# Yasas1994/Jaeger

Measured on AMD Instinct MI355X. Metric: Mbp/s classified (1500bp frags), higher is better.
Workload: dtype f16x3 (split-f16, f32 accumulate)

## Files before the change

include/jaeger_hip.h:

```cpp
#ifndef JAEGER_HIP_H
#define JAEGER_HIP_H

#include <stdint.h>

#ifdef __cplusplus
extern "C" {
#endif

#define JG_ABI_VERSION 1
#define JG_MAX_STAGES 8
#define JG_MAX_BUFS 6
#define JG_MAX_VECS 12

typedef enum {
  JG_OK = 0,
  JG_ERR_INVALID = -1,
  JG_ERR_HIP = -2,
  JG_ERR_UNSUPPORTED = -3,
  JG_ERR_NOMEM = -4,
  JG_ERR_IO = -5
} jg_status;

enum { JG_PTR_HOST = 0, JG_PTR_DEVICE = 1 };

// ... 59 lines not shown
  int32_t padding;
  int32_t mask_mode;
  int32_t in_vec, out_vec;
  int32_t vec_off;
  int32_t arg;
  int64_t w_off;
  int64_t b_off;
  float f0;
  int32_t n_stages;
  jg_stage stages[JG_MAX_STAGES];
} jg_op;

typedef struct jg_engine jg_engine;
typedef struct jg_model jg_model;

int jg_abi_version(void);
int jg_sizeof(int which);
const char *jg_last_error(void);
int jg_engine_create(int device_id, jg_engine **out);
int jg_engine_destroy(jg_engine *e);
int jg_engine_sync(jg_engine *e);
enum { JG_OPT_STREAM_BYTES = 1, JG_OPT_CONV_PC = 2, JG_OPT_TERMINI_EXACT = 3, JG_OPT_DUST_ON_COPY_STREAM = 4,
       JG_OPT_TABLE_NET_LDS = 5, JG_OPT_RESET_PROGRESS = 6, JG_OPT_FUSE_RESBLOCK = 7, JG_OPT_TERMINI_REPORT_MIN = 8,
       JG_OPT_STREAM_PRIORITY = 9 };
int jg_engine_set_option(jg_engine *e, int key, int64_t value);
enum { JG_STAT_STREAM_GROUPS = 1, JG_STAT_STREAM_BYTES = 2, JG_STAT_PEAK_DEVICE_BASES = 3, JG_STAT_DUST_MASKED = 4,
       JG_STAT_WINDOWS_DONE = 5 };
int64_t jg_engine_get_stat(const jg_engine *e, int key);
int jg_engine_set_dust(jg_engine *e, const int64_t *rec_off, int64_t n_records, int32_t window, int32_t threshold);

int jg_model_create(jg_engine *e, const jg_op *ops, int n_ops, const float *weights,
                    int64_t n_weights, int32_t vocab, jg_model **out);
int jg_model_destroy(jg_model *m);
int jg_model_set_precision(jg_model *m, int mode);
int jg_model_get_precision(const jg_model *m);
enum { JG_MSTAT_CONVS = 0, JG_MSTAT_CONVS_F16X3 = 1, JG_MSTAT_LAYOUT_CONVERSIONS = 2, JG_MSTAT_SMALL_FUSED = 3,
       JG_MSTAT_TAP_VARIANT = 4 };
int64_t jg_model_get_stat(const jg_model *m, int key);
enum { JG_TAP_F16S = 1, JG_TAP_PHASE_SPLIT = 2, JG_TAP_WINDOW_PACKED = 4, JG_TAP_TABLE_LOOKUP = 8, JG_TAP_NARROW = 16,
       JG_TAP_EXACT_F32 = 32, JG_TAP_FUSED_RESBLOCK = 64 };
int jg_model_tap_shape(const jg_model *m, int op, int32_t l, int64_t shape[4]);
int jg_model_set_tap(jg_model *m, int op, void *host_dst, int64_t dst_bytes);
int jg_model_describe(const jg_model *m, char *buf, int64_t cap);

enum { JG_ENC_PRECASED = 1, JG_ENC_CASE_SENSITIVE = 2, JG_ENC_NUCLEOTIDE = 4, JG_ENC_DICODON = 8 };
int jg_encode(jg_engine *e, const uint8_t *bases, int64_t n_bases, int bases_loc,
              const int64_t *win_start, const int32_t *win_len, int win_loc, int64_t n_win,
              int32_t fsize, const uint8_t *lut65, int32_t soft_mask, int32_t l_pad,
              uint8_t *ids, int32_t *counts, int out_loc, void *stream);

int jg_forward(jg_model *m, const uint8_t *ids, int ids_loc, int64_t n_win, int32_t l,
               float *prediction, float *reliability, float *embedding, float *nmd,
               int out_loc, int32_t chunk, void *stream);

int jg_predict_windows(jg_model *m, const uint8_t *bases, int64_t n_bases, int bases_loc,
                       const int64_t *win_start, const int32_t *win_len, int win_loc,
                       int64_t n_win, int32_t fsize, const uint8_t *lut65, int32_t soft_mask,
                       int32_t l_pad, float *prediction, float *reliability, float *embedding,
                       float *nmd, int32_t *counts, int out_loc, int32_t chunk, void *stream);

// ... 64 lines not shown
```

jaeger_amd/_lib.py:

```python

from __future__ import annotations

import ctypes as C
import os
from pathlib import Path

JG_MAX_STAGES = 8
JG_MAX_BUFS = 6
JG_MAX_VECS = 12
JG_PTR_HOST, JG_PTR_DEVICE = 0, 1
JG_BUF_NONE, JG_BUF_IDS = -1, -2
JG_OK, JG_ERR_INVALID, JG_ERR_HIP, JG_ERR_UNSUPPORTED, JG_ERR_NOMEM, JG_ERR_IO = 0, -1, -2, -3, -4, -5
JG_OPT_STREAM_BYTES = 1
JG_OPT_CONV_PC = 2
JG_OPT_TERMINI_EXACT = 3
JG_OPT_TERMINI_REPORT_MIN = 8
JG_OPT_DUST_ON_COPY_STREAM = 4
JG_OPT_TABLE_NET_LDS = 5
JG_OPT_RESET_PROGRESS = 6
JG_OPT_FUSE_RESBLOCK = 7
JG_OPT_STREAM_PRIORITY = 9
JG_COL_STRING, JG_COL_INT, JG_COL_FLOAT, JG_COL_BOOL, JG_COL_SPANS = 0, 1, 2, 3, 4
JG_STAT_STREAM_GROUPS, JG_STAT_STREAM_BYTES, JG_STAT_PEAK_DEVICE_BASES, JG_STAT_DUST_MASKED, JG_STAT_WINDOWS_DONE = 1, 2, 3, 4, 5
JG_MSTAT_CONVS, JG_MSTAT_CONVS_F16X3, JG_MSTAT_LAYOUT_CONVERSIONS, JG_MSTAT_SMALL_FUSED = 0, 1, 2, 3
JG_MSTAT_TAP_VARIANT = 4
JG_PROF_MFMA_F16X3, JG_PROF_MFMA_F32, JG_PROF_TABLE, JG_PROF_FUSED_SMALL, JG_PROF_FRAMEATTN, JG_PROF_FRAMEATTN_CVT = range(6)
TAP_F16S, TAP_PHASE_SPLIT, TAP_WINDOW_PACKED, TAP_TABLE_LOOKUP, TAP_NARROW, TAP_EXACT_F32, TAP_FUSED_RESBLOCK = 1, 2, 4, 8, 16, 32, 64

OP_CONV, OP_MASK, OP_POOL, OP_DENSE, OP_ELTWISE, OP_NMD_FINAL, OP_OODSIG, OP_MAXPOOL1D, OP_FRAMESUM, OP_STRANDS, OP_EMBED, OP_VECMAX, OP_FRAMEATTN = range(1, 14)
ST_NONE, ST_BIAS, ST_BN, ST_DYT, ST_ADD, ST_ACT, ST_NMD, ST_MASKMUL, ST_LN = range(9)
ACT_NONE, ACT_GELU_TANH, ACT_GELU_ERF, ACT_RELU, ACT_TANH, ACT_SIGMOID = range(6)
MASK_ANY, MASK_MAJORITY, MASK_STRICT = range(3)
PAD_VALID, PAD_SAME = 0, 1
POOL_MAX, POOL_AVG, POOL_MAX_NOMASK = 0, 1, 2
MERGE_AVERAGE, MERGE_SUM, MERGE_MAX, MERGE_CONCAT = 0, 1, 2, 3
JG_ENC_PRECASED, JG_ENC_CASE_SENSITIVE, JG_ENC_NUCLEOTIDE, JG_ENC_DICODON = 1, 2, 4, 8
VEC_EMBEDDING, VEC_NMD, VEC_PREDICTION, VEC_RELIABILITY, VEC_SCRATCH0 = 0, 1, 2, 3, 4


class JgStage(C.Structure):
    _fields_ = [("kind", C.c_int32), ("arg", C.c_int32),
                ("p0", C.c_int64), ("p1", C.c_int64), ("p2", C.c_int64), ("p3", C.c_int64),
                ("f0", C.c_float), ("pad_", C.c_int32)]


class JgOp(C.Structure):
    _fields_ = [("kind", C.c_int32), ("in_buf", C.c_int32), ("out_buf", C.c_int32),
                ("in_mask", C.c_int32), ("out_mask", C.c_int32),
# ... 117 lines not shown
```

jaeger_amd/csrc/jg_api.hip:

```cpp
#include <stdarg.h>
#include <stdio.h>
#include <string.h>

#include <algorithm>
#include <string>
#include <thread>

#include "jg_common.h"
#include "jg_small.h"
#include "jg_resblock64.h"
#include "jg_vecmax.h"
#include "jg_frameattn.h"

static thread_local char g_err[1024] = "";

void jg_set_error(const char *fmt, ...) {
  va_list ap;
  va_start(ap, fmt);
  vsnprintf(g_err, sizeof(g_err), fmt, ap);
  va_end(ap);
}

extern "C" const char *jg_last_error(void) { return g_err; }
extern "C" int jg_abi_version(void) { return JG_ABI_VERSION; }
// ... 66 lines not shown
#ifndef JG_EXPERIMENT
      JG_REQUIRE(value == 0, JG_ERR_UNSUPPORTED, "jg_engine_set_option: JG_OPT_CONV_PC = %lld needs the experiment build (make -C jaeger_amd/csrc "
                 "exp; JAEGER_HIP_LIB=jaeger_amd/libjaeger_hip_exp.so): the producer / consumer kernels are not in the shipped library",
                 (long long)value);
#endif
      e->conv_pc = (int)value;
      return JG_OK;
    case JG_OPT_TERMINI_EXACT:
      e->termini_exact = value != 0;
      return JG_OK;
    case JG_OPT_TERMINI_REPORT_MIN:
      JG_REQUIRE(value == 0 || (value >= 2 && value <= 15), JG_ERR_INVALID,
                 "jg_engine_set_option: JG_OPT_TERMINI_REPORT_MIN = %lld (0, or 2 .. 15 columns)", (long long)value);
      e->termini_report_min = (int)value;
      return JG_OK;
    case JG_OPT_DUST_ON_COPY_STREAM:
      e->dust_on_copy = value != 0;
      return JG_OK;
    case JG_OPT_TABLE_NET_LDS:
      e->tab_lds_only = value != 0;
      return JG_OK;
    case JG_OPT_FUSE_RESBLOCK:
      e->fuse_resblock = value != 0;
      return JG_OK;
    case JG_OPT_RESET_PROGRESS:
      e->windows_done.store(0, std::memory_order_release);
      return JG_OK;
    case JG_OPT_STREAM_PRIORITY: {
      JG_REQUIRE(value == 0 || value == 1, JG_ERR_INVALID, "jg_engine_set_option: JG_OPT_STREAM_PRIORITY takes 0 or 1, got %lld",
                 (long long)value);
      JG_HIP(hipSetDevice(e->dev));
      JG_HIP(hipStreamSynchronize(e->stream));
      int least = 0, greatest = 0;
      JG_HIP(hipDeviceGetStreamPriorityRange(&least, &greatest));
      hipStream_t fresh = nullptr;
      JG_HIP(hipStreamCreateWithPriority(&fresh, hipStreamNonBlocking, value ? greatest : least));
      (void)hipStreamDestroy(e->stream);
      e->stream = fresh;
      return JG_OK;
    }
    default:
      jg_set_error("jg_engine_set_option: unknown key %d", key);
      return JG_ERR_INVALID;
  }
}

// ... 1337 lines not shown
    out += line;
  }
  const size_t n = std::min(out.size(), (size_t)cap - 1);
  memcpy(buf, out.data(), n);
  buf[n] = 0;
  return JG_OK;
}

extern "C" int64_t jg_model_get_stat(const jg_model *m, int key) {
  if (m == nullptr) return -1;
  int64_t n_conv = 0, n_f16 = 0, n_cvt = 0;
  for (size_t i = 0; i < m->ops.size(); ++i) {
    n_cvt += m->hprep[i].n_cvt;
    if (m->ops[i].kind != JG_OP_CONV) continue;
    ++n_conv;
    n_f16 += (m->f16_eligible && m->hprep[i].f16_ok) ? 1 : 0;
  }
  switch (key) {
    case JG_MSTAT_CONVS: return n_conv;
    case JG_MSTAT_CONVS_F16X3: return n_f16;
    case JG_MSTAT_LAYOUT_CONVERSIONS: return m->f16_eligible ? n_cvt : 0;
    case JG_MSTAT_SMALL_FUSED: return m->small != nullptr ? 1 : 0;
    case JG_MSTAT_TAP_VARIANT: return m->tap_variant;
    default: return -1;
  }
}

extern "C" int jg_model_destroy(jg_model *m);
extern "C" int jg_model_create(jg_engine *e, const jg_op *ops, int n_ops, const float *weights,
                               int64_t n_weights, int32_t vocab, jg_model **out) {
  JG_REQUIRE(e != nullptr && ops != nullptr && n_ops > 0 && weights != nullptr && n_weights > 0 &&
                 out != nullptr,
             JG_ERR_INVALID, "jg_model_create: bad arguments");
  JG_HIP(hipSetDevice(e->dev));
  jg_model *m = new jg_model();
  m->e = e;
  m->ops.assign(ops, ops + n_ops);
  m->n_w = n_weights;
  m->vocab = vocab;
  int rc = validate_program(m);
  if (rc != JG_OK) { delete m; return rc; }
  if (m->ops[0].kind == JG_OP_EMBED && m->vocab > 256) m->id_bytes = 2;
  if (m->ops.back().kind == JG_OP_STRANDS) {
    m->strands = m->ops.back().k;
    m->id_frames = 1;
    m->merge_kind = m->ops.back().arg;
// ... 493 lines not shown
              a.wh = hp.d_wh_ps[in.L & 1];
              a.tap_lo = 1; a.tap_hi = 3;
              a.pad_left = 1 + a.tap_lo * a.dil;
            } else {
              a.tap_lo = a.tap_hi = 2;
              a.pad_left = 0 + a.tap_lo * a.dil;
            }
          }
          a.psplit = hp.ps_store ? 1 : 0;
          a.L_res = eff_stride == 2 ? 2 * lo - 1 : lo;
          a.tiles_m = (a.L_res + jg_conv_f16_tile_m() - 1) / jg_conv_f16_tile_m();
          const int strips = hp.cw == 128 ? 2 : 4;
          int strips_per_win = in.frames * a.tiles_m * strips;
          {
            static const bool no_flat = jg_exp_env("JG_NO_FLAT") != nullptr;
            const int halo = (a.k - 1) * a.dil;
            const int gap = std::max(a.pad_left, halo - a.pad_left);
            const int fp = lo + gap;
            const bool strip_rows = hp.nmd_slot >= 0 || hp.nmd_slot2 >= 0 || hp.pool_op >= 0;
            const int wp_unit = strip_rows ? 128 : 32;
            const int wp = (in.frames * fp + wp_unit - 1) / wp_unit * wp_unit;
            const int64_t flat_tiles = ((int64_t)nw * wp + 255) / 256;
            const int64_t row_tiles = (int64_t)a.rows * a.tiles_m;
            if (!no_flat && a.k == 5 && op.in_buf != JG_BUF_IDS && hp.d_lut == nullptr && eff_stride == 1 && eff_lin == lo &&
                ((op.cout == 128 && !hp.as_k5 && hp.ps_read == 0 && !hp.ps_store) ? jg_conv_f16_has_flat_pattern(hp.ep) : jg_conv_f16_has_narrow_pattern(hp.ep)) &&
                (int64_t)nw * wp < (1 << 24) && flat_tiles * 100 <= row_tiles * 95) {
              a.flat = 1;
              a.flat_p = fp;
              a.flat_wp = wp;
              a.flat_frames = in.frames;
              a.flat_tiles = (int)flat_tiles;
              a.flat_inv_p = 1.0f / (float)fp;
              a.flat_inv_wp = 1.0f / (float)wp;
              strips_per_win = wp / (256 / strips);
              m->tap_flat = 1;
            }
          }
          if (hp.nmd_slot >= 0) m->part_rows[hp.nmd_slot] = strips_per_win;
          if (hp.nmd_slot2 >= 0) m->part_rows[hp.nmd_slot2] = strips_per_win;
          if (hp.pool_op >= 0) m->pool_rows = strips_per_win;
          a.out_f16s = hp.out_f16s ? 1 : 0;
          a.act_kind = hp.act_kind;
          a.n_hst = hp.n_hst;
          a.ep = hp.ep;
          a.alpha1 = hp.alpha1; a.alpha2 = hp.alpha2;
          a.dytmask1 = hp.dytmask1; a.dytmask2 = hp.dytmask2;
          a.n_epi_rows = hp.n_epi_rows;
          a.epi = hp.d_epi;
          for (int q = 0; q < hp.n_hst; ++q) a.hst[q] = hp.hst[q];
          if (hp.add_slot >= 0) a.addh = reinterpret_cast<const uint4 *>(m->act[hp.add_slot]);
          if (hp.nmd_slot >= 0) a.nmd_out = m->nmd_part[hp.nmd_slot];
          if (hp.nmd_slot2 >= 0) a.nmd_out2 = m->nmd_part[hp.nmd_slot2];
          a.ep_rt = hp.ep_rt;
          if (hp.pool_op >= 0) {
            const int64_t need = (int64_t)a.rows * a.tiles_m * strips * op.cout;
            if (need > m->pool_part_cap) {
              JG_HIP(hipStreamSynchronize(s));
              if (m->pool_part) (void)hipFree(m->pool_part);
// ... 258 lines not shown
      return rc;
    if (m->precision != 1) break;
    int flag = 0;
    JG_HIP(hipMemcpyAsync(&flag, m->d_overflow, sizeof(int), hipMemcpyDeviceToHost, s));
    JG_HIP(hipStreamSynchronize(s));
    if (flag == 0) break;
    JG_HIP(hipMemsetAsync(m->d_overflow, 0, sizeof(int), s));
    m->precision = 0;
    m->f16_reason = "an activation left the f16 range at run time";
  }
  return JG_OK;
}

extern "C" int jg_forward(jg_model *m, const uint8_t *ids, int ids_loc, int64_t n_win, int32_t l,
                          float *prediction, float *reliability, float *embedding, float *nmd,
                          int out_loc, int32_t chunk, void *stream) {
  JG_REQUIRE(m != nullptr && ids != nullptr && n_win >= 0 && l > 0, JG_ERR_INVALID,
             "jg_forward: bad arguments");
  if (n_win == 0) return JG_OK;
  jg_engine *e = m->e;
  JG_HIP(hipSetDevice(e->dev));
  hipStream_t s = pick_stream(e, stream);
  m->tap_variant = 0;
  const uint8_t *d_ids = ids;
  if (ids_loc == JG_PTR_HOST) {
    const int64_t bytes = n_win * m->strands * m->id_frames * (int64_t)l * m->id_bytes;
    int rc = grow(&m->d_ids, &m->d_ids_cap, bytes);
    if (rc != JG_OK) return rc;
    JG_HIP(hipMemcpyAsync(m->d_ids, ids, (size_t)bytes, hipMemcpyHostToDevice, s));
    d_ids = m->d_ids;
  }
  int rc = forward_device_ids(m, d_ids, n_win, l, prediction, reliability, embedding, nmd, out_loc,
                              chunk, s);
  if (rc != JG_OK) return rc;
  if (out_loc == JG_PTR_HOST || ids_loc == JG_PTR_HOST) JG_HIP(hipStreamSynchronize(s));
  return JG_OK;
}

static int frame_len(int nt) {
  if (nt < 3) return 0;
  const int off = (nt % 3 == 0) ? -2 : ((nt % 3 == 1) ? -1 : 0);
  const int usable = nt - 5 + off;
  return usable > 0 ? (usable + 2) / 3 : 0;
}

static int encode_common(jg_engine *e, jg_model *scratch_owner, const uint8_t *bases, int64_t n_bases,
// ... 428 lines not shown
```

jaeger_amd/csrc/jg_common.h:

```cpp
#pragma once
#include <hip/hip_runtime.h>
#include <stdint.h>
#include <atomic>
#include <string>
#include <vector>

#include "jaeger_hip.h"

void jg_set_error(const char *fmt, ...);

#include <stdlib.h>
static inline const char *jg_exp_env(const char *name) {
#ifdef JG_EXPERIMENT
  return getenv(name);
#else
  (void)name;
  return nullptr;
#endif
}

#define JG_HIP(call)                                                                 \
  do {                                                                               \
    hipError_t err_ = (call);                                                        \
    if (err_ != hipSuccess) {                                                        \
// ... 128 lines not shown
struct ProfEvent {
  hipEvent_t a, b;
  double flops;
  int cls = 0;
};

struct jg_engine {
  int dev = 0;
  hipStream_t stream = nullptr;
  hipEvent_t t0 = nullptr, t1 = nullptr;
  bool profile = false;
  std::vector<ProfEvent> pending;
  std::vector<hipEvent_t> pool;
  double conv_ms = 0.0, conv_flops = 0.0;
  int64_t conv_launches = 0;
  double cls_ms[JG_PROF_CLASSES] = {}, cls_flops[JG_PROF_CLASSES] = {};
  int64_t cls_launches[JG_PROF_CLASSES] = {};
  int n_cu = 256;
  int dust_on_copy = 1;
  int termini_exact = 0;
  int termini_report_min = 0;
  int tab_lds_only = 0;
  int fuse_resblock = 1;
  int conv_pc = 0;
  int64_t stream_bytes = (int64_t)32 << 20;
  hipStream_t copy_stream = nullptr;
  void *pin[2] = {nullptr, nullptr};
  void *dbase[2] = {nullptr, nullptr};
  int64_t pin_cap = 0, dbase_cap = 0;
  hipEvent_t h2d_done[2] = {nullptr, nullptr};
  hipEvent_t enc_done[2] = {nullptr, nullptr};
  hipEvent_t grp_done[2] = {nullptr, nullptr};
  void *pin_io[2] = {nullptr, nullptr};
  int64_t pin_io_cap = 0;
  std::atomic<int64_t> windows_done{0};
  int64_t streamed_groups = 0, streamed_bytes = 0, peak_dev_bases = 0;
  int64_t *d_rec_off = nullptr;
  int64_t rec_cap = 0, n_rec = 0, rec_end = 0;
  int dust_window = 0, dust_threshold = 0;
  unsigned long long *d_dust_cnt = nullptr;
};

struct ConvHPrep {
  uint4 *d_wh = nullptr;
  int n_half = 1;
  int cw = 128;
// ... 69 lines not shown
  uint8_t *d_lut = nullptr;
  float *pool_part = nullptr;
  int64_t pool_part_cap = 0;
  std::vector<int> pool_fused_by;
  int strands = 1;
  int id_frames = 6;
  int id_bytes = 1;
  int merge_kind = 0;
  float *merged[JG_MAX_VECS] = {};
  int64_t merged_cap[JG_MAX_VECS] = {};
  float *tab_table = nullptr;
  float *tab_bias = nullptr;
  int tab_conv = -1, tab_pool = -1;
  uint16_t *tab_wfrag = nullptr;
  float *tab_bias512 = nullptr;
  int tab_act = 0, tab_cq = 0, tab_vocab = 0, tab_zero = 0;
  int part_rows[JG_MAX_BUFS] = {};
  int pool_rows = 0;
  int tap_op = -1;
  void *tap_dst = nullptr;
  int64_t tap_bytes = 0;
  int64_t tap_row0 = 0;
  int64_t tap_variant = 0;
  int tap_flat = 0;
  float *tap_buf = nullptr;
  int64_t tap_cap = 0;
};

int jg_usable_cores();

int jg_launch_conv(jg_engine *e, const ConvArgs &a, hipStream_t s);
int jg_launch_embed(const uint16_t *ids, int64_t n_pos, const float *table, int vocab, int c, float *out, uint8_t *mask,
                    hipStream_t s);
int jg_launch_mask(const uint8_t *in, int rows, int L_in, int L_out, int k, int stride, int dil,
                   int pad_left, int mode, uint8_t *out, hipStream_t s);
int jg_launch_pool(const float *x, const uint8_t *mask, int n_win, int positions, int c, int kind,
                   float *out, int out_ld, hipStream_t s);
int jg_launch_dense(const float *in, int in_ld, const float *w, const float *b, int n_win, int cin,
                    int cout, int act, float *out, int out_ld, hipStream_t s);
int jg_launch_nmd_final(const float *part, int parts_per_win, const uint8_t *mask, int positions,
                        const float *moving_mean, float eps, int n_win, int c, float *out,
                        int out_ld, int out_off, hipStream_t s);
int jg_launch_eltwise(const EltArgs &a, hipStream_t s);
int jg_launch_layernorm(const EltArgs &a, int rows, int L, int tiles_m, hipStream_t s);
int jg_launch_encode(const uint8_t *bases, const int64_t *win_start, const int32_t *win_len,
                     int64_t n_win, int fsize, const uint8_t *lut, int flags, int l_pad,
// ... 47 lines not shown
```

jaeger_amd/csrc/jg_conv_dev.h:

```cpp
#pragma once
#include "jg_common.h"

typedef float f32x16 __attribute__((ext_vector_type(16)));
typedef _Float16 half8 __attribute__((ext_vector_type(8)));
typedef _Float16 half4 __attribute__((ext_vector_type(4)));

namespace {

constexpr int HM = 256;
constexpr int HN = 128;
constexpr int HT = 256;
constexpr int NT = 1;
constexpr int A_ITERS = 5;
constexpr int W_ITERS = 2;
constexpr int W_ITEMS = 2 * 2 * HN;
constexpr int LUT_RS = 68;

__device__ __forceinline__ float fast_gelu(float v) {
  const float t = v * (-2.3022082f - 0.10294324f * v * v);
  return v * __builtin_amdgcn_rcpf(1.0f + __builtin_amdgcn_exp2f(t));
}
typedef float f32x2 __attribute__((ext_vector_type(2)));
__device__ __forceinline__ f32x2 fast_gelu2(f32x2 v) {
  const f32x2 c2 = {0.10294324f, 0.10294324f}, c1 = {-2.3022082f, -2.3022082f}, one = {1.0f, 1.0f};
// ... 57 lines not shown
template <int N>
__device__ __forceinline__ void wait_vm() {
  asm volatile("s_waitcnt vmcnt(%0)" ::"n"(N) : "memory");
}

template <int H>
__device__ __forceinline__ float mix_sum(unsigned hi2, unsigned lo2) {
  float r;
  if constexpr (H == 0) asm("v_fma_mix_f32 %0, %1, 1.0, %2 op_sel:[0,0,0] op_sel_hi:[1,0,1]" : "=v"(r) : "v"(hi2), "v"(lo2));
  else asm("v_fma_mix_f32 %0, %1, 1.0, %2 op_sel:[1,0,1] op_sel_hi:[1,0,1]" : "=v"(r) : "v"(hi2), "v"(lo2));
  return r;
}
template <int H>
__device__ __forceinline__ float mix_rem(float v, unsigned hi2) {
  float r;
  if constexpr (H == 0) asm("v_fma_mix_f32 %0, %1, -1.0, %2 op_sel:[0,0,0] op_sel_hi:[1,0,0]" : "=v"(r) : "v"(hi2), "v"(v));
  else asm("v_fma_mix_f32 %0, %1, -1.0, %2 op_sel:[1,0,0] op_sel_hi:[1,0,0]" : "=v"(r) : "v"(hi2), "v"(v));
  return r;
}

struct Tile {
  int rowblk, m0, valid;
  int T;
};

__device__ __forceinline__ void udivmod24(int v, int d, float inv, int &q, int &r) {
  q = (int)((float)v * inv);
  r = v - q * d;
  if (r < 0) { --q; r += d; }
  else if (r >= d) { ++q; r -= d; }
}

}
```

jaeger_amd/csrc/jg_conv_f16_impl.h:

```cpp
#include <stdio.h>
#include <stdlib.h>
#include <type_traits>

#include "jg_common.h"

#include "jg_conv_dev.h"

namespace {


#ifdef JG_STAMP
static __device__ unsigned long long jg_stamp_acc[8];
#define JG_ST_DECL unsigned long long st_[8] = {0, 0, 0, 0, 0, 0, 0, 0}; unsigned long long st_t = __builtin_amdgcn_s_memtime(); const unsigned long long st_t0 = st_t
#define JG_ST(idx) do { const unsigned long long n_ = __builtin_amdgcn_s_memtime(); st_[idx] += n_ - st_t; st_t = n_; } while (0)
#define JG_ST_END do { st_[5] = __builtin_amdgcn_s_memtime() - st_t0; if (lane == 0) { for (int q_ = 0; q_ < 8; ++q_) atomicAdd(&jg_stamp_acc[q_], st_[q_]); } } while (0)
#else
#define JG_ST_DECL
#define JG_ST(idx)
#define JG_ST_END
#endif

#ifndef JG_PRIO
#define JG_PRIO 1
#endif
// ... 27 lines not shown
  const int wm = LUT ? (wid & 1) : (NARROW ? wid : (wid >> 1));
  const int wn = LUT ? ((GEN && a.lut_one_half) ? 0 : (int)(blockIdx.x & 1u)) : (NARROW ? 0 : (wid & 1));
  const int i = lane & 31, h = lane >> 5;
  const int lut_sh = (LUT && !(GEN && a.lut_one_half)) ? 1 : 0;
  const int vgrid = (int)(gridDim.x >> lut_sh);
  int vb = (int)(blockIdx.x >> lut_sh);
  if ((vgrid & 7) == 0) vb = (vb & 7) * (vgrid >> 3) + (vb >> 3);
  constexpr int TPER = LUT ? JG_LUT_WAVES / 2 : NT;
  const int tsub = LUT ? (wid >> 1) : 0;
  const int rows_a = HM + (K - 1) * a.dil;
  const int a_items = NT * 4 * rows_a;
  uint4 *Abuf = lds;
  uint4 *Wbuf = lds + 2 * a_items;
  const int lut_rows = a.k * (a.lut_vocab + 1);
  float *epiL = LUT ? reinterpret_cast<float *>(lds) + lut_rows * LUT_RS
                    : reinterpret_cast<float *>(Wbuf + K * W_ITEMS);
  for (int q = tid; q < a.n_epi_rows * 2 * HN; q += NTHR) epiL[q] = a.epi[q];
  const unsigned lds0 = (unsigned)(size_t)(__attribute__((address_space(3))) void *)lds;
  const unsigned ldsA = __builtin_amdgcn_readfirstlane(lds0 + wid * 1024);
  const unsigned ldsW = __builtin_amdgcn_readfirstlane(lds0 + 2 * a_items * 16 + wid * 1024);

  const int n_tiles = FLAT ? a.flat_tiles : a.rows * a.tiles_m;
  const int n_pairs = (n_tiles + TPER - 1) / TPER;
  auto resolve = [&](const Tile &tile, int local, int len, int &row, int &p) -> bool {
    if constexpr (!FLAT) {
      row = tile.rowblk;
      p = tile.m0 + local;
      return tile.valid && p >= 0 && p < len;
    }
    const int v = tile.T * HM + local;
    if (v < 0 || !tile.valid) { row = 0; p = 0; return false; }
    int g, u, f;
    udivmod24(v, a.flat_wp, a.flat_inv_wp, g, u);
    udivmod24(u, a.flat_p, a.flat_inv_p, f, p);
    row = g * a.flat_frames + f;
    return f < a.flat_frames && p < len && row < a.rows;
  };
  int my_pairs = 0;
  if (vb < n_pairs) my_pairs = (n_pairs - 1 - vb) / vgrid + 1;
  if (my_pairs == 0) return;

  unsigned a_pk[A_ITERS];
#pragma unroll
  for (int it = 0; it < A_ITERS; ++it) {
    const int q = tid + it * HT;
    const int ph = q / rows_a;
    a_pk[it] = ((unsigned)(ph >> 2) << 20) | ((unsigned)(ph & 3) << 16) | (unsigned)(q - ph * rows_a);
  }
  unsigned w_voff[W_ITERS];
#pragma unroll
  for (int it = 0; it < W_ITERS; ++it) {
    const int q = tid + it * HT;
    w_voff[it] = (unsigned)((((q >> 8) * K * a.cc_in * 2 + ((q >> 7) & 1)) * HN + (q & (HN - 1))) * 16);
  }

  auto tiles_of = [&](int pass, Tile *t) {
#pragma unroll
    for (int u = 0; u < NT; ++u) {
      const int T = (vb + pass * vgrid) * TPER + tsub + u;
      const int Tc = min(T, n_tiles - 1);
      t[u].rowblk = Tc / a.tiles_m;
      t[u].m0 = (Tc - t[u].rowblk * a.tiles_m) * HM;
      t[u].valid = T < n_tiles;
      t[u].T = Tc;
    }
  };

  const uint8_t *bsrc = a.ids != nullptr ? a.ids : a.mask_in;
  unsigned char raw[A_ITERS];
  unsigned x_voff[A_ITERS];
  unsigned x_ok = 0;
  auto piece_pos = [&](const Tile *tl2, int it, int &pc, bool &inr) -> int {
    const int a_u = (int)(a_pk[it] >> 20), a_r = (int)(a_pk[it] & 0xffff);
    int rb, p;
    inr = resolve(tl2[0], a_r - a.pad_left, a.L_in, rb, p) && a_u < NT;
    pc = min(max(p, 0), a.L_in - 1);
    if constexpr (FLAT) rb = min(rb, a.rows - 1);
    return rb;
  };
  auto load_bytes = [&](const Tile *tl2) {
    if (bsrc != nullptr) {
#pragma unroll
      for (int it = 0; it < A_ITERS; ++it) {
        int pc; bool inr;
        const int rb = piece_pos(tl2, it, pc, inr);
        raw[it] = bsrc[(size_t)rb * a.L_in + pc];
      }
    } else {
#pragma unroll
      for (int it = 0; it < A_ITERS; ++it) raw[it] = 1;
    }
  };
  auto build_pieces = [&](const Tile *tl2) {
    x_ok = 0;
#pragma unroll
    for (int it = 0; it < A_ITERS; ++it) {
      int pc; bool inr;
      const int rb = piece_pos(tl2, it, pc, inr);
      const unsigned ph = (a_pk[it] >> 16) & 3;
      const unsigned byte = raw[it];
// ... 677 lines not shown
          if (!live) row = min(max(row, 0), a.rows - 1);
        }
        return live;
      };
      constexpr bool OPOS = !GEN;
      unsigned ob[TM], om[TM], olive = 0;
      size_t o_row = 0, o_mrow = 0;
      unsigned o_step = 0;
      const void *e_y = a.y, *e_addh = a.addh;
      const uint8_t *e_mask = a.mask_out;
      int e_dbg = a.dbg, e_f16s = a.out_f16s;
      float *e_pool = a.pool_out, *e_nmd = a.nmd_out;
      int *e_overflow = a.overflow;
      if constexpr (OPOS) {
        typedef const __attribute__((address_space(4))) ConvHArgs *KArgs;
        KArgs ka = (KArgs)__builtin_amdgcn_kernarg_segment_ptr();
        asm volatile("" : "+s"(ka));
        e_addh = ka->addh;
        e_mask = ka->mask_out;
        e_dbg = ka->dbg;
        e_f16s = ka->out_f16s;
        e_nmd = ka->nmd_out;
        const unsigned Lo = (unsigned)ka->L_out, CC4 = (unsigned)(ka->cout_pad >> 4) * 4u;
        o_step = FLAT ? 2u * Lo : 32u * Lo;
        asm volatile("" : "+s"(o_step));
        if constexpr (!FLAT) {
          o_row = (size_t)cur[0].rowblk * CC4 * Lo * 16u + (size_t)(wn * 8) * o_step;
          o_mrow = (size_t)cur[0].rowblk * Lo;
        }
#pragma unroll
        for (int tm = 0; tm < TM; ++tm) {
          int row, p;
          const bool live = resolve(cur[0], (wm * TM + tm) * 32 + i, (int)Lo, row, p);
          const int mc = live ? p : 0;
          if constexpr (FLAT) {
            if (!live) row = min(max(row, 0), a.rows - 1);
          }
          if (live) olive |= 1u << tm;
          if constexpr (FLAT) {
            om[tm] = (unsigned)row * Lo + (unsigned)mc;
            ob[tm] = ((unsigned)row * CC4 + (unsigned)h) * Lo + (unsigned)mc;
          } else {
            om[tm] = (unsigned)mc;
            ob[tm] = ((unsigned)h * Lo + (unsigned)mc) * 16u;
          }
        }
      }
      auto o_item = [&](const void *base, int tm, int tn, int j, int plane) -> const char * {
        if constexpr (FLAT) {
          return reinterpret_cast<const char *>(base) + ((size_t)(ob[tm] + (unsigned)(((wn * 2 + tn) * 2 + j) * 2 + plane) * o_step) << 4);
        } else {
          return reinterpret_cast<const char *>(base) + (o_row + (size_t)((unsigned)((tn * 2 + j) * 2 + plane) * o_step)) + ob[tm];
        }
      };
      auto o_maskbyte = [&](int tm) -> unsigned char {
        return e_mask != nullptr ? (e_mask + o_mrow)[om[tm]] : (unsigned char)1;
      };
      auto prefetch = [&](Pre &p, const Tile &tile, int tm, int tn) {
        const int nb = (wn * 2 + tn) * 32;
        int orow = 0, mc = 0;
        if constexpr (OPOS) {
          p.mkb = o_maskbyte(tm);
        } else {
          out_pos(tile, tm, orow, mc);
          p.mkb = a.mask_out != nullptr ? a.mask_out[(size_t)orow * a.L_out + mc] : (unsigned char)1;
        }
        if (e_addh != nullptr && !(e_dbg & 128)) {
#pragma unroll
          for (int j = 0; j < 2; ++j) {
            typedef unsigned u32x4 __attribute__((ext_vector_type(4)));
            const u32x4 *src_h, *src_l;
            if constexpr (OPOS) {
              src_h = reinterpret_cast<const u32x4 *>(o_item(e_addh, tm, tn, j, 0));
              src_l = reinterpret_cast<const u32x4 *>(o_item(e_addh, tm, tn, j, 1));
            } else {
              const unsigned it4 = item4(orow, mc, (!GEN || nb + ch0 + 16 * j < a.cout) ? nb : 0, j);
// ... 165 lines not shown
            x[4 * j + 2] = __uint_as_float(h2); x[4 * j + 3] = __uint_as_float(h3);
            x[8 + 4 * j + 0] = __uint_as_float(l0); x[8 + 4 * j + 1] = __uint_as_float(l1);
            x[8 + 4 * j + 2] = __uint_as_float(l2); x[8 + 4 * j + 3] = __uint_as_float(l3);
          }
        }
      };
      char *f32_base = nullptr;
      auto store_block = [&](const f32x16 &x, const Tile &tile, int tm, int tn, bool f16s) {
        const int nb = (wn * 2 + tn) * 32;
        if constexpr (OPOS) {
          typedef unsigned u32x4 __attribute__((ext_vector_type(4)));
          if (f16s) {
#pragma unroll
            for (int j = 0; j < 2; ++j) {
              const u32x4 vhi = {__float_as_uint(x[4 * j]), __float_as_uint(x[4 * j + 1]),
                                 __float_as_uint(x[4 * j + 2]), __float_as_uint(x[4 * j + 3])};
              const u32x4 vlo = {__float_as_uint(x[8 + 4 * j]), __float_as_uint(x[8 + 4 * j + 1]),
                                 __float_as_uint(x[8 + 4 * j + 2]), __float_as_uint(x[8 + 4 * j + 3])};
              st_stream(vhi, reinterpret_cast<u32x4 *>(const_cast<char *>(o_item(e_y, tm, tn, j, 0))));
              st_stream(vlo, reinterpret_cast<u32x4 *>(const_cast<char *>(o_item(e_y, tm, tn, j, 1))));
            }
          } else {
            char *yf = f32_base + tn * (32 * 4);
            if constexpr (FLAT) yf += ((size_t)om[tm] * (HN * 4) + 16 * h);
            else yf += om[tm] * (unsigned)(HN * 4) + 16u * (unsigned)h;
#pragma unroll
            for (int g = 0; g < 4; ++g)
              *reinterpret_cast<float4 *>(yf + 32 * g) = make_float4(x[4 * g], x[4 * g + 1], x[4 * g + 2], x[4 * g + 3]);
          }
          return;
        }
        int orow, mc;
        const bool live = out_pos(tile, tm, orow, mc);
        if (live && !(e_dbg & 64)) {
          if (e_f16s) {
            uint4 *yh = reinterpret_cast<uint4 *>(a.y);
#pragma unroll
            for (int j = 0; j < 2; ++j) {
              if (GEN && nb + ch0 + 16 * j >= a.cout) continue;
              const unsigned it4 = item4_out(orow, mc, nb, j);
              typedef unsigned u32x4 __attribute__((ext_vector_type(4)));
              const u32x4 vhi = {__float_as_uint(x[4 * j]), __float_as_uint(x[4 * j + 1]),
                                 __float_as_uint(x[4 * j + 2]), __float_as_uint(x[4 * j + 3])};
              const u32x4 vlo = {__float_as_uint(x[8 + 4 * j]), __float_as_uint(x[8 + 4 * j + 1]),
                                 __float_as_uint(x[8 + 4 * j + 2]), __float_as_uint(x[8 + 4 * j + 3])};
              st_stream(vhi, reinterpret_cast<u32x4 *>(yh + it4));
              st_stream(vlo, reinterpret_cast<u32x4 *>(yh + it4 + 2u * (unsigned)L_st));
              if (GEN && psplit && (a.L_out & 1) && mc == a.L_out - 1) {
// ... 388 lines not shown
```

jaeger_amd/engine.py:

```python

from __future__ import annotations

import ctypes as C
import weakref
from collections import defaultdict
from pathlib import Path
from typing import Any, Iterable

import numpy as np
import yaml

from . import _lib as L
from .plan import ModelPlan, build_plan
from .program import Program, compile_plan


def _yaml_load(text: str):
    loader = getattr(yaml, "CSafeLoader", None)
    return yaml.load(text, Loader=loader) if loader is not None else yaml.safe_load(text)


def frame_length(nucleotides: int) -> int:
    nt = int(nucleotides)
    if nt < 3:
# ... 46 lines not shown

    __del__ = close

    def sync(self):
        L.check(self.lib.jg_engine_sync(self.handle), "jg_engine_sync")

    def set_stream_bytes(self, nbytes: int):
        L.check(self.lib.jg_engine_set_option(self.handle, L.JG_OPT_STREAM_BYTES, int(nbytes)), "jg_engine_set_option")

    def set_stream_priority(self, high: bool):
        L.check(self.lib.jg_engine_set_option(self.handle, L.JG_OPT_STREAM_PRIORITY, int(bool(high))), "jg_engine_set_option")

    def set_table_net_lds(self, on: bool):
        L.check(self.lib.jg_engine_set_option(self.handle, L.JG_OPT_TABLE_NET_LDS, int(bool(on))), "jg_engine_set_option")

    def set_conv_pc(self, on: bool):
        L.check(self.lib.jg_engine_set_option(self.handle, L.JG_OPT_CONV_PC, int(on)), "jg_engine_set_option")

    def windows_done(self) -> int:
        return int(self.lib.jg_engine_get_stat(self.handle, L.JG_STAT_WINDOWS_DONE))

    def set_fuse_resblock(self, on: bool):
        L.check(self.lib.jg_engine_set_option(self.handle, L.JG_OPT_FUSE_RESBLOCK, int(bool(on))), "jg_engine_set_option")

    def reset_progress(self):
        L.check(self.lib.jg_engine_set_option(self.handle, L.JG_OPT_RESET_PROGRESS, 0), "jg_engine_set_option")

    def stream_stats(self) -> dict:
        g = lambda k: int(self.lib.jg_engine_get_stat(self.handle, k))
        return {"groups": g(L.JG_STAT_STREAM_GROUPS), "bytes": g(L.JG_STAT_STREAM_BYTES),
                "peak_device_bases": g(L.JG_STAT_PEAK_DEVICE_BASES)}

    def alloc(self, nbytes: int) -> int:
        p = C.c_void_p()
        L.check(self.lib.jg_dev_alloc(self.handle, int(nbytes), C.byref(p)), "jg_dev_alloc")
        return p.value or 0

    def free(self, ptr: int):
        if ptr:
            L.check(self.lib.jg_dev_free(self.handle, C.c_void_p(ptr)), "jg_dev_free")

    def upload(self, arr: np.ndarray) -> int:
        arr = np.ascontiguousarray(arr)
        p = self.alloc(max(arr.nbytes, 1))
        L.check(self.lib.jg_memcpy_h2d(self.handle, C.c_void_p(p), _ptr(arr), arr.nbytes), "jg_memcpy_h2d")
        return p
# ... 137 lines not shown
        o = self._host_outputs(n, want)
        L.check(self.lib.jg_forward(self.handle, _ptr(ids), L.JG_PTR_HOST, n, l, _ptr(o["prediction"]),
                                    _ptr(o["reliability"]), _ptr(o["embedding"]), _ptr(o["nmd"]),
                                    L.JG_PTR_HOST, int(chunk), None), "jg_forward")
        return {k: v for k, v in o.items() if v is not None}

    def tap(self, op: int, ids: np.ndarray, chunk: int = 0) -> np.ndarray:
        ids = np.ascontiguousarray(ids, np.uint16 if self.wide_ids else np.uint8)
        shape = (C.c_int64 * 4)()
        L.check(self.lib.jg_model_tap_shape(self.handle, int(op), ids.shape[2], shape), "jg_model_tap_shape")
        rows, frames, l_out, c = (int(v) for v in shape)
        is_mask = self.program.ops[op].kind == L.OP_MASK
        out = np.zeros((ids.shape[0] * rows, frames, l_out) if is_mask else (ids.shape[0] * rows, frames, l_out, c),
                       np.uint8 if is_mask else np.float32)
        L.check(self.lib.jg_model_set_tap(self.handle, int(op), _ptr(out), out.nbytes), "jg_model_set_tap")
        try:
            self.forward(ids, chunk=chunk, want=())
        finally:
            self.lib.jg_model_set_tap(self.handle, -1, None, 0)
        return out

    def tap_variant(self) -> int:
        return int(self.lib.jg_model_get_stat(self.handle, L.JG_MSTAT_TAP_VARIANT))

    def predict_windows(self, bases, n_bases: int, win_start, win_len, n_win: int, fsize: int, lut,
                        flags: int = 0, l_pad: int | None = None, chunk: int = 0, device_inputs=False,
                        want=("prediction", "reliability", "embedding", "nmd"), counts=True, out: dict | None = None):
        l_pad = self.row_length(fsize) if l_pad is None else int(l_pad)
        res = out if out is not None else self.host_outputs(n_win, want, counts)
        o = {k: res.get(k) for k in ("prediction", "reliability", "embedding", "nmd")}
        cnt = res.get("counts")
        loc = L.JG_PTR_DEVICE if device_inputs else L.JG_PTR_HOST
        lut = np.ascontiguousarray(lut, np.uint8)
        L.check(self.lib.jg_predict_windows(
            self.handle, _ptr(bases), int(n_bases), loc, _ptr(win_start), _ptr(win_len), loc, int(n_win),
            int(fsize), _ptr(lut), int(flags), l_pad, _ptr(o["prediction"]), _ptr(o["reliability"]),
            _ptr(o["embedding"]), _ptr(o["nmd"]), _ptr(cnt), L.JG_PTR_HOST, int(chunk), None),
            "jg_predict_windows")
        return res

    def host_outputs(self, n_win: int, want=("prediction", "reliability", "embedding", "nmd"), counts=True) -> dict:
        self.dev.reset_progress()
        res = {k: v for k, v in self._host_outputs(n_win, want).items() if v is not None}
        if counts:
            res["counts"] = np.zeros((n_win, 4), np.int32)
        return res
# ... 136 lines not shown
```

Measured before the change: 85.59.

## Precompute flat-tile window/frame coordinates and simplify packed conv output addressing

Adds a window_packed engine option (default 1) that keeps the existing flat-tile selection heuristic and exposes alternative modes and a packed-launch counter. Inside the f16 conv kernel, flat tiles now carry precomputed window base, frame index and distance-to-window-end. When frames are long enough, the per-element row and position are resolved with cheap comparisons instead of divisions. Flat-mode output addressing is rewritten to use a per-tile row base plus small relative offsets, sharing the non-flat epilogue path. This is meant to cut integer address arithmetic in the epilogue and loader. The new index math is more complex and could mis-resolve rows near window boundaries.

```diff
diff --git a/include/jaeger_hip.h b/include/jaeger_hip.h
--- a/include/jaeger_hip.h
+++ b/include/jaeger_hip.h
@@ -105,7 +105,7 @@
 int jg_engine_sync(jg_engine *e);
 enum { JG_OPT_STREAM_BYTES = 1, JG_OPT_CONV_PC = 2, JG_OPT_TERMINI_EXACT = 3, JG_OPT_DUST_ON_COPY_STREAM = 4,
        JG_OPT_TABLE_NET_LDS = 5, JG_OPT_RESET_PROGRESS = 6, JG_OPT_FUSE_RESBLOCK = 7, JG_OPT_TERMINI_REPORT_MIN = 8,
-       JG_OPT_STREAM_PRIORITY = 9 };
+       JG_OPT_STREAM_PRIORITY = 9, JG_OPT_WINDOW_PACKED = 10 };
 int jg_engine_set_option(jg_engine *e, int key, int64_t value);
 enum { JG_STAT_STREAM_GROUPS = 1, JG_STAT_STREAM_BYTES = 2, JG_STAT_PEAK_DEVICE_BASES = 3, JG_STAT_DUST_MASKED = 4,
        JG_STAT_WINDOWS_DONE = 5 };
@@ -118,7 +118,7 @@
 int jg_model_set_precision(jg_model *m, int mode);
 int jg_model_get_precision(const jg_model *m);
 enum { JG_MSTAT_CONVS = 0, JG_MSTAT_CONVS_F16X3 = 1, JG_MSTAT_LAYOUT_CONVERSIONS = 2, JG_MSTAT_SMALL_FUSED = 3,
-       JG_MSTAT_TAP_VARIANT = 4 };
+       JG_MSTAT_TAP_VARIANT = 4, JG_MSTAT_PACKED_LAUNCHES = 5 };
 int64_t jg_model_get_stat(const jg_model *m, int key);
 enum { JG_TAP_F16S = 1, JG_TAP_PHASE_SPLIT = 2, JG_TAP_WINDOW_PACKED = 4, JG_TAP_TABLE_LOOKUP = 8, JG_TAP_NARROW = 16,
        JG_TAP_EXACT_F32 = 32, JG_TAP_FUSED_RESBLOCK = 64 };
diff --git a/jaeger_amd/_lib.py b/jaeger_amd/_lib.py
--- a/jaeger_amd/_lib.py
+++ b/jaeger_amd/_lib.py
@@ -20,10 +20,12 @@
 JG_OPT_RESET_PROGRESS = 6
 JG_OPT_FUSE_RESBLOCK = 7
 JG_OPT_STREAM_PRIORITY = 9
+JG_OPT_WINDOW_PACKED = 10
 JG_COL_STRING, JG_COL_INT, JG_COL_FLOAT, JG_COL_BOOL, JG_COL_SPANS = 0, 1, 2, 3, 4
 JG_STAT_STREAM_GROUPS, JG_STAT_STREAM_BYTES, JG_STAT_PEAK_DEVICE_BASES, JG_STAT_DUST_MASKED, JG_STAT_WINDOWS_DONE = 1, 2, 3, 4, 5
 JG_MSTAT_CONVS, JG_MSTAT_CONVS_F16X3, JG_MSTAT_LAYOUT_CONVERSIONS, JG_MSTAT_SMALL_FUSED = 0, 1, 2, 3
 JG_MSTAT_TAP_VARIANT = 4
+JG_MSTAT_PACKED_LAUNCHES = 5
 JG_PROF_MFMA_F16X3, JG_PROF_MFMA_F32, JG_PROF_TABLE, JG_PROF_FUSED_SMALL, JG_PROF_FRAMEATTN, JG_PROF_FRAMEATTN_CVT = range(6)
 TAP_F16S, TAP_PHASE_SPLIT, TAP_WINDOW_PACKED, TAP_TABLE_LOOKUP, TAP_NARROW, TAP_EXACT_F32, TAP_FUSED_RESBLOCK = 1, 2, 4, 8, 16, 32, 64
 
diff --git a/jaeger_amd/csrc/jg_api.hip b/jaeger_amd/csrc/jg_api.hip
--- a/jaeger_amd/csrc/jg_api.hip
+++ b/jaeger_amd/csrc/jg_api.hip
@@ -112,6 +112,10 @@
       return JG_OK;
     case JG_OPT_FUSE_RESBLOCK:
       e->fuse_resblock = value != 0;
+      return JG_OK;
+    case JG_OPT_WINDOW_PACKED:
+      JG_REQUIRE(value >= 0 && value <= 3, JG_ERR_INVALID, "jg_engine_set_option: JG_OPT_WINDOW_PACKED takes 0 .. 3, got %lld", (long long)value);
+      e->window_packed = (int)value;
       return JG_OK;
     case JG_OPT_RESET_PROGRESS:
       e->windows_done.store(0, std::memory_order_release);
@@ -1495,6 +1499,7 @@
     case JG_MSTAT_LAYOUT_CONVERSIONS: return m->f16_eligible ? n_cvt : 0;
     case JG_MSTAT_SMALL_FUSED: return m->small != nullptr ? 1 : 0;
     case JG_MSTAT_TAP_VARIANT: return m->tap_variant;
+    case JG_MSTAT_PACKED_LAUNCHES: return m->packed_launches;
     default: return -1;
   }
 }
@@ -2034,9 +2039,17 @@
             const int wp = (in.frames * fp + wp_unit - 1) / wp_unit * wp_unit;
             const int64_t flat_tiles = ((int64_t)nw * wp + 255) / 256;
             const int64_t row_tiles = (int64_t)a.rows * a.tiles_m;
+            bool take = flat_tiles * 100 <= row_tiles * 95;
+            if (!take && !strip_rows && e->window_packed == 3) {
+              const int64_t wgs = 2 * (int64_t)e->n_cu;
+              const int64_t grid_f = std::min(wgs, flat_tiles), grid_r = std::min(wgs, row_tiles);
+              take = (flat_tiles + grid_f - 1) / grid_f < (row_tiles + grid_r - 1) / grid_r;
+            }
+            if (e->window_packed == 2) take = flat_tiles <= row_tiles;
+            if (e->window_packed == 0) take = false;
             if (!no_flat && a.k == 5 && op.in_buf != JG_BUF_IDS && hp.d_lut == nullptr && eff_stride == 1 && eff_lin == lo &&
                 ((op.cout == 128 && !hp.as_k5 && hp.ps_read == 0 && !hp.ps_store) ? jg_conv_f16_has_flat_pattern(hp.ep) : jg_conv_f16_has_narrow_pattern(hp.ep)) &&
-                (int64_t)nw * wp < (1 << 24) && flat_tiles * 100 <= row_tiles * 95) {
+                (int64_t)nw * wp < (1 << 24) && take) {
               a.flat = 1;
               a.flat_p = fp;
               a.flat_wp = wp;
@@ -2046,6 +2059,7 @@
               a.flat_inv_wp = 1.0f / (float)wp;
               strips_per_win = wp / (256 / strips);
               m->tap_flat = 1;
+              m->packed_launches += hp.n_half;
             }
           }
           if (hp.nmd_slot >= 0) m->part_rows[hp.nmd_slot] = strips_per_win;
@@ -2350,6 +2364,7 @@
   JG_HIP(hipSetDevice(e->dev));
   hipStream_t s = pick_stream(e, stream);
   m->tap_variant = 0;
+  m->packed_launches = 0;
   const uint8_t *d_ids = ids;
   if (ids_loc == JG_PTR_HOST) {
     const int64_t bytes = n_win * m->strands * m->id_frames * (int64_t)l * m->id_bytes;
diff --git a/jaeger_amd/csrc/jg_common.h b/jaeger_amd/csrc/jg_common.h
--- a/jaeger_amd/csrc/jg_common.h
+++ b/jaeger_amd/csrc/jg_common.h
@@ -174,6 +174,7 @@
   int termini_report_min = 0;
   int tab_lds_only = 0;
   int fuse_resblock = 1;
+  int window_packed = 1;
   int conv_pc = 0;
   int64_t stream_bytes = (int64_t)32 << 20;
   hipStream_t copy_stream = nullptr;
@@ -289,6 +290,7 @@
   int64_t tap_bytes = 0;
   int64_t tap_row0 = 0;
   int64_t tap_variant = 0;
+  int64_t packed_launches = 0;
   int tap_flat = 0;
   float *tap_buf = nullptr;
   int64_t tap_cap = 0;
diff --git a/jaeger_amd/csrc/jg_conv_dev.h b/jaeger_amd/csrc/jg_conv_dev.h
--- a/jaeger_amd/csrc/jg_conv_dev.h
+++ b/jaeger_amd/csrc/jg_conv_dev.h
@@ -103,6 +103,7 @@
 struct Tile {
   int rowblk, m0, valid;
   int T;
+  int f0, dw;
 };
 
 __device__ __forceinline__ void udivmod24(int v, int d, float inv, int &q, int &r) {
diff --git a/jaeger_amd/csrc/jg_conv_f16_impl.h b/jaeger_amd/csrc/jg_conv_f16_impl.h
--- a/jaeger_amd/csrc/jg_conv_f16_impl.h
+++ b/jaeger_amd/csrc/jg_conv_f16_impl.h
@@ -73,11 +73,20 @@
 
   const int n_tiles = FLAT ? a.flat_tiles : a.rows * a.tiles_m;
   const int n_pairs = (n_tiles + TPER - 1) / TPER;
+  const bool flat_near = FLAT && CW == 128 && a.flat_p >= HM + (K - 1) * a.dil;
   auto resolve = [&](const Tile &tile, int local, int len, int &row, int &p) -> bool {
     if constexpr (!FLAT) {
       row = tile.rowblk;
       p = tile.m0 + local;
       return tile.valid && p >= 0 && p < len;
+    }
+    if (FLAT && CW == 128 && flat_near) {
+      int t = tile.m0 + local, f = tile.f0, rb = tile.rowblk;
+      if (local >= tile.dw) { rb += a.flat_frames; f = 0; t = local - tile.dw; }
+      else if (t >= a.flat_p) { ++f; t -= a.flat_p; }
+      row = rb + f;
+      p = t;
+      return tile.valid && t >= 0 && f < a.flat_frames && t < len && row < a.rows;
     }
     const int v = tile.T * HM + local;
     if (v < 0 || !tile.valid) { row = 0; p = 0; return false; }
@@ -110,8 +119,16 @@
     for (int u = 0; u < NT; ++u) {
       const int T = (vb + pass * vgrid) * TPER + tsub + u;
       const int Tc = min(T, n_tiles - 1);
-      t[u].rowblk = Tc / a.tiles_m;
-      t[u].m0 = (Tc - t[u].rowblk * a.tiles_m) * HM;
+      if constexpr (FLAT) {
+        const int g0 = (Tc * HM) / a.flat_wp, u0 = Tc * HM - g0 * a.flat_wp;
+        t[u].rowblk = g0 * a.flat_frames;
+        t[u].f0 = u0 / a.flat_p;
+        t[u].m0 = u0 - t[u].f0 * a.flat_p;
+        t[u].dw = a.flat_wp - u0;
+      } else {
+        t[u].rowblk = Tc / a.tiles_m;
+        t[u].m0 = (Tc - t[u].rowblk * a.tiles_m) * HM;
+      }
       t[u].valid = T < n_tiles;
       t[u].T = Tc;
     }
@@ -126,7 +143,7 @@
     int rb, p;
     inr = resolve(tl2[0], a_r - a.pad_left, a.L_in, rb, p) && a_u < NT;
     pc = min(max(p, 0), a.L_in - 1);
-    if constexpr (FLAT) rb = min(rb, a.rows - 1);
+    if constexpr (FLAT) rb = min(max(rb, 0), a.rows - 1);
     return rb;
   };
   auto load_bytes = [&](const Tile *tl2) {
@@ -850,24 +867,20 @@
         e_f16s = ka->out_f16s;
         e_nmd = ka->nmd_out;
         const unsigned Lo = (unsigned)ka->L_out, CC4 = (unsigned)(ka->cout_pad >> 4) * 4u;
-        o_step = FLAT ? 2u * Lo : 32u * Lo;
+        o_step = 32u * Lo;
         asm volatile("" : "+s"(o_step));
-        if constexpr (!FLAT) {
-          o_row = (size_t)cur[0].rowblk * CC4 * Lo * 16u + (size_t)(wn * 8) * o_step;
-          o_mrow = (size_t)cur[0].rowblk * Lo;
-        }
+        o_row = (size_t)cur[0].rowblk * CC4 * Lo * 16u + (size_t)(wn * 8) * o_step;
+        o_mrow = (size_t)cur[0].rowblk * Lo;
 #pragma unroll
         for (int tm = 0; tm < TM; ++tm) {
           int row, p;
           const bool live = resolve(cur[0], (wm * TM + tm) * 32 + i, (int)Lo, row, p);
           const int mc = live ? p : 0;
-          if constexpr (FLAT) {
-            if (!live) row = min(max(row, 0), a.rows - 1);
-          }
           if (live) olive |= 1u << tm;
           if constexpr (FLAT) {
-            om[tm] = (unsigned)row * Lo + (unsigned)mc;
-            ob[tm] = ((unsigned)row * CC4 + (unsigned)h) * Lo + (unsigned)mc;
+            const unsigned rel = live ? (unsigned)(row - cur[0].rowblk) : 0u;
+            om[tm] = rel * Lo + (unsigned)mc;
+            ob[tm] = ((rel * CC4 + (unsigned)h) * Lo + (unsigned)mc) * 16u;
           } else {
             om[tm] = (unsigned)mc;
             ob[tm] = ((unsigned)h * Lo + (unsigned)mc) * 16u;
@@ -875,11 +888,7 @@
         }
       }
       auto o_item = [&](const void *base, int tm, int tn, int j, int plane) -> const char * {
-        if constexpr (FLAT) {
-          return reinterpret_cast<const char *>(base) + ((size_t)(ob[tm] + (unsigned)(((wn * 2 + tn) * 2 + j) * 2 + plane) * o_step) << 4);
-        } else {
-          return reinterpret_cast<const char *>(base) + (o_row + (size_t)((unsigned)((tn * 2 + j) * 2 + plane) * o_step)) + ob[tm];
-        }
+        return reinterpret_cast<const char *>(base) + (o_row + (size_t)((unsigned)((tn * 2 + j) * 2 + plane) * o_step)) + ob[tm];
       };
       auto o_maskbyte = [&](int tm) -> unsigned char {
         return e_mask != nullptr ? (e_mask + o_mrow)[om[tm]] : (unsigned char)1;
@@ -1091,8 +1100,7 @@
             }
           } else {
             char *yf = f32_base + tn * (32 * 4);
-            if constexpr (FLAT) yf += ((size_t)om[tm] * (HN * 4) + 16 * h);
-            else yf += om[tm] * (unsigned)(HN * 4) + 16u * (unsigned)h;
+            yf += om[tm] * (unsigned)(HN * 4) + 16u * (unsigned)h;
 #pragma unroll
             for (int g = 0; g < 4; ++g)
               *reinterpret_cast<float4 *>(yf + 32 * g) = make_float4(x[4 * g], x[4 * g + 1], x[4 * g + 2], x[4 * g + 3]);
diff --git a/jaeger_amd/engine.py b/jaeger_amd/engine.py
--- a/jaeger_amd/engine.py
+++ b/jaeger_amd/engine.py
@@ -92,6 +92,9 @@
 
     def set_fuse_resblock(self, on: bool):
         L.check(self.lib.jg_engine_set_option(self.handle, L.JG_OPT_FUSE_RESBLOCK, int(bool(on))), "jg_engine_set_option")
+
+    def set_window_packed(self, mode: int):
+        L.check(self.lib.jg_engine_set_option(self.handle, L.JG_OPT_WINDOW_PACKED, int(mode)), "jg_engine_set_option")
 
     def reset_progress(self):
         L.check(self.lib.jg_engine_set_option(self.handle, L.JG_OPT_RESET_PROGRESS, 0), "jg_engine_set_option")
@@ -275,6 +278,9 @@
 
     def tap_variant(self) -> int:
         return int(self.lib.jg_model_get_stat(self.handle, L.JG_MSTAT_TAP_VARIANT))
+
+    def packed_launches(self) -> int:
+        return int(self.lib.jg_model_get_stat(self.handle, L.JG_MSTAT_PACKED_LAUNCHES))
 
     def predict_windows(self, bases, n_bases: int, win_start, win_len, n_win: int, fsize: int, lut,
                         flags: int = 0, l_pad: int | None = None, chunk: int = 0, device_inputs=False,
```

Measured after the change: 85.71 (median of 2 runs). Within noise of the previous version (+0.1%).
